# JVBSouza/descriptools

Hardware: AMD Instinct MI355X
Metric: Mcells/s full descriptor chain (higher is better)
Workload: dtype f32; 1 GPU; 16384x16384 synthetic tilted-integer-fBm DEM per GPU, full chain (d8, flowacc, river mask, flowhand/HAND with fused GFI + ln(hl/H), fused slope+TI+MTI, downslope), device-resident; global_dem=16384x16384, river_threshold_cells=524288

## Files before the change

### descriptools_amd/csrc/dt_fa3fh1_kernel.inc

```
#if FA3_WALK
#define FA3_NAME(n) n##w
#define FA3_NAME_TWI(n) n##w_twi
#else
#define FA3_NAME(n) n
#define FA3_NAME_TWI(n) n##_twi
#endif
#if FA3_TWI
__global__ __launch_bounds__(256, 6) void FA3_NAME_TWI(k_fa3fh1)(const uint8_t *__restrict__ fdr, const float *__restrict__ dem,
#else
template <int ND>
__global__ __launch_bounds__(256, 6) void FA3_NAME(k_fa3fh1)(const uint8_t *__restrict__ fdr, const float *__restrict__ dem,
#endif
                                                  const uint8_t *__restrict__ nod4, int ldm, DtWin w, int tiles_x,
                                                  const unsigned long long *__restrict__ rec,
                                                  const unsigned long long *__restrict__ state,
                                                  const unsigned long long *__restrict__ ext,
                                                  const uint16_t *__restrict__ loc16, int32_t *__restrict__ acc32,
                                                  int32_t river_thr, int8_t *__restrict__ river,
                                                  int *__restrict__ status, uint32_t nnodes,
                                                  unsigned long long *__restrict__ nodes,
                                                  unsigned long long *__restrict__ cache,
#if FA3_TWI
                                                  uint8_t *__restrict__ cache_wide, TwiOut tw) {
  constexpr int ND = 2;
#else
                                                  uint8_t *__restrict__ cache_wide) {
#endif
#undef FA3_NAME
#undef FA3_NAME_TWI
#define P3(c) ((uint32_t)(c) + (((uint32_t)(c) >> 6) << 2))
#define NT3 (TH * (TW + 4))
  __shared__ __attribute__((aligned(16))) unsigned char smem[NT3 * 6];
  __shared__ unsigned long long s_in;
#if !FA3_WALK
  __shared__ int s_ovf;
#endif
  uint32_t *s_delta = reinterpret_cast<uint32_t *>(smem);
  uint16_t *s_nxt = reinterpret_cast<uint16_t *>(smem + NT3 * 4);
  const int tile = dt_tile_of_block((int)blockIdx.x, (int)gridDim.x);
  const int ty = tile / tiles_x, tx = tile - ty * tiles_x;
  const int y0 = ty * TH, x0 = tx * TW;
  const uint4 v_fdr = dt_tile_fetch16(fdr, w, y0, x0);
  uint32_t c2[8] = {0u, 0u, 0u, 0u, 0u, 0u, 0u, 0u};
  if (rec) fa_nbr_codes(fdr, w, y0, x0, threadIdx.x, c2);
  unsigned long long e = 0ull;
  if (threadIdx.x < PS && ext) e = ext[(size_t)tile * PS + threadIdx.x];
  constexpr int VPT = NT / 4 / 256;
  uint2 l4[VPT];
  float4 z4[VPT];
#if FA3_TWI
  fa_v4f s4[VPT];
#endif
#pragma unroll
  for (int u = 0; u < VPT; u++) {
    int c = 4 * (threadIdx.x + 256 * u);
    int y = y0 + c / TW;
    l4[u] = *reinterpret_cast<const uint2 *>(loc16 + (size_t)tile * NT + c);
    z4[u] = make_float4(0.f, 0.f, 0.f, 0.f);
#if FA3_TWI
    s4[u] = (fa_v4f){0.f, 0.f, 0.f, 0.f};
    if (y < w.H)
      s4[u] = __builtin_nontemporal_load(reinterpret_cast<const fa_v4f *>(tw.slope + (long long)y * w.ld + x0 + c % TW));
#endif
    if (ND == 1 && y < w.H) z4[u] = *reinterpret_cast<const float4 *>(dem + (long long)y * w.ld + x0 + c % TW);
    if (ND == 2 && y < w.H) {
      const uint32_t m = (uint32_t)reinterpret_cast<const uint16_t *>(nod4)[(long long)(y >> 2) * ldm + ((x0 + c % TW) >> 2)] >>
                         (4 * (y & 3));
      z4[u] = make_float4((m & 1u) ? DT_NODATA : 0.f, (m & 2u) ? DT_NODATA : 0.f, (m & 4u) ? DT_NODATA : 0.f,
                          (m & 8u) ? DT_NODATA : 0.f);
    }
  }
  {
    const int ly = (int)threadIdx.x >> 2, lxb = ((int)threadIdx.x & 3) * 16;
    const uint32_t cv[4] = {v_fdr.x, v_fdr.y, v_fdr.z, v_fdr.w};
    const bool interior = dt_tile_interior(w, y0, x0);
    const int pbase = ly * (TW + 4) + lxb;
#pragma unroll
    for (int q = 0; q < 4; q++) {
      uint32_t nn[4];
#pragma unroll
      for (int k = 0; k < 4; k++) {
        const uint32_t code = (cv[q] >> (8 * k)) & 0xFFu;
        const int lx = lxb + 4 * q + k;
        const uint32_t n = interior ? dt_tile_next_interior(code, ly, lx) : dt_tile_next(code, ly, lx, y0, x0, w);
        nn[k] = n < NT ? P3(n) : n;
      }
      *reinterpret_cast<uint2 *>(&s_nxt[pbase + 4 * q]) = make_uint2(nn[0] | (nn[1] << 16), nn[2] | (nn[3] << 16));
      *reinterpret_cast<uint4 *>(&s_delta[pbase + 4 * q]) = make_uint4(0, 0, 0, 0);
    }
  }
  if (rec) e = fa_inflow(fa_gather(c2, y0, x0, threadIdx.x, tiles_x, rec, state), e);
#if FA3_WALK
  bool fed_now = false;
#pragma unroll
  for (int q = 0; q < 8; q++) fed_now = fed_now || c2[q] == fa_back(q);
  const unsigned long long fed_mask = __ballot(fed_now);
#endif
#if !FA3_WALK
  if (threadIdx.x == 0) s_ovf = 0;
#endif
  if (__syncthreads_or(!(e & FA_CYCLE) && FA_VALUE(e) >= (1ull << 22))) {
    if (threadIdx.x == 0) s_in = 0ull;
    __syncthreads();
    if (e != 0ull && !(e & FA_CYCLE)) atomicAdd(&s_in, FA_VALUE(e));
    __syncthreads();
    if (threadIdx.x == 0 && s_in >= (1ull << 31) - (unsigned long long)NT && status) atomicOr(status, DT_STATUS_ACC_OVERFLOW);
  }
  if (e != 0ull) {
    int ly, lx;
    dt_cell_of_slot(threadIdx.x, ly, lx);
    uint32_t c = P3(ly * TW + lx);
    if (e & FA_CYCLE) {
      for (int it = 0; it < NT && c < NT3; it++) {
        atomicOr(&s_delta[c], 0x80000000u);
        c = s_nxt[c];
      }
    } else {
      const uint32_t add = (uint32_t)e;
      for (int it = 0; it < NT && c < NT3; it++) {
        atomicAdd(&s_delta[c], add);
        c = s_nxt[c];
      }
    }
  }
  __syncthreads();
  auto finish = [&](uint32_t l16, uint32_t d, float z) -> int32_t {
    int32_t v = l16 == 0xFFFFu ? -100 : (int32_t)l16;
    if (v != -100) v += (int32_t)(d & 0x7FFFFFFFu);
    if (d & 0x80000000u) v = -100;
    if (ND != 0 && z <= DT_NODATA) v = -100;
    return v;
  };
  uint32_t riv4[VPT];
#pragma unroll
  for (int u = 0; u < VPT; u++) {
    int c = 4 * (threadIdx.x + 256 * u);
    int y = y0 + c / TW;
    riv4[u] = 0u;
    if (y >= w.H) continue;
    long long o = (long long)y * w.ld + x0 + c % TW;
    uint4 d = *reinterpret_cast<const uint4 *>(&s_delta[P3(c)]);
    int4 v = make_int4(finish(l4[u].x & 0xFFFFu, d.x, z4[u].x), finish(l4[u].x >> 16, d.y, z4[u].y),
                       finish(l4[u].y & 0xFFFFu, d.z, z4[u].z), finish(l4[u].y >> 16, d.w, z4[u].w));
    *reinterpret_cast<int4 *>(acc32 + o) = v;
    riv4[u] = (v.x > river_thr ? 1u : 0u) | (v.y > river_thr ? 0x100u : 0u) | (v.z > river_thr ? 0x10000u : 0u) |
              (v.w > river_thr ? 0x1000000u : 0u);
    *reinterpret_cast<uint32_t *>(river + o) = riv4[u];
#if FA3_TWI
    {
      const int32_t fv[4] = {v.x, v.y, v.z, v.w};
      const double nlnpx2 = tw.n_top * tw.lnpx2;
      fa_v4f tio, mtio;
      uint32_t rej = 0u;
#pragma unroll
      for (int k = 0; k < 4; k++) {
        const float q = dt_pct_to_tan(s4[u][k]);
        const bool tnod = fv[k] <= -100;
        float tv, mv;
        rej |= ((sd_twi_fast(fv[k], q, tw.n_top, tw.lnpx2, nlnpx2, tv, mv) && !tnod) ? 1u : 0u) << k;
        tio[k] = tnod ? DT_NODATA : tv;
        mtio[k] = tnod ? DT_NODATA : mv;
      }
      __builtin_nontemporal_store(tio, reinterpret_cast<fa_v4f *>(tw.ti + o));
      __builtin_nontemporal_store(mtio, reinterpret_cast<fa_v4f *>(tw.mti + o));
      if (rej) {
        const int x = x0 + c % TW;
        const int stile = (y >> 4) * tw.stiles_x + (x >> 8);
        const size_t lane = (size_t)stile * 256 + (size_t)(((y & 15) >> 2) * 64 + ((x & 255) >> 2));
        atomicOr(&tw.lane_mask[lane >> 1], rej << (16 * (int)(lane & 1) + 4 * (y & 3)));
        tw.tile_mark[stile] = (uint8_t)1;
      }
    }
#endif
  }
#if FA3_WALK
#pragma unroll
  for (int u = 0; u < VPT; u++) {
    if (!riv4[u]) continue;
    const uint32_t pc = P3(4 * (threadIdx.x + 256 * u));
    uint2 nx = *reinterpret_cast<const uint2 *>(&s_nxt[pc]);
    if (riv4[u] & 0x1u) nx.x = (nx.x & 0xFFFF0000u) | NX_RIVER;
    if (riv4[u] & 0x100u) nx.x = (nx.x & 0xFFFFu) | (NX_RIVER << 16);
    if (riv4[u] & 0x10000u) nx.y = (nx.y & 0xFFFF0000u) | NX_RIVER;
    if (riv4[u] & 0x1000000u) nx.y = (nx.y & 0xFFFFu) | (NX_RIVER << 16);
    *reinterpret_cast<uint2 *>(&s_nxt[pc]) = nx;
  }
#endif
  __syncthreads();
#if FA3_WALK
  fh_walk_body(s_nxt, fdr, ((fed_mask >> (threadIdx.x & 63u)) & 1ull) != 0ull, w, tile, tiles_x, y0, x0, nodes, cache_wide);
#undef P3
#undef NT3
}
#else
#undef P3
#undef NT3
  uint32_t *s_w = reinterpret_cast<uint32_t *>(smem);
  uint8_t *s_fdr = smem + NT * 4;
  uint8_t *s_kind = smem + NT * 5;
  uint32_t *s_lut = reinterpret_cast<uint32_t *>(smem + NT * 6);
  s_lut[threadIdx.x] = fh_lut_entry(threadIdx.x);
  dt_tile_put16(s_fdr, v_fdr);
  __syncthreads();
  fh_tile1n_body(s_fdr, s_w, s_kind, &s_ovf, s_lut, riv4, w, tile, tiles_x, y0, x0, nnodes, nodes, cache, cache_wide);
}
#endif
```

### descriptools_amd/csrc/dt_tiles.hip

```cpp
#include "dt_common.h"
#include "dt_kernels.h"
#include "dt_math.h"

#define TW 64
#define TH 64
#define NT (TW * TH)
#define PS (2 * TW + 2 * (TH - 2))
#define CPT (NT / 256)

#define NX_SINK 0xFFFFu
#define NX_EXIT 0xFFFEu
#define NX_REXIT 0xFFFDu
#define X_NONE 0xFFFFu

__device__ __forceinline__ int dt_slot_of(int ly, int lx) {
  if (ly == 0) return lx;
  if (ly == TH - 1) return TW + lx;
  if (lx == 0) return 2 * TW + (ly - 1);
  if (lx == TW - 1) return 2 * TW + (TH - 2) + (ly - 1);
  return -1;
}
__device__ __forceinline__ void dt_cell_of_slot(int s, int &ly, int &lx) {
  if (s < TW) { ly = 0; lx = s; }
  else if (s < 2 * TW) { ly = TH - 1; lx = s - TW; }
// ... 1122 lines not shown
      if (y >= w.H || x >= w.W || code == 0u) {
        s = fht_pack((uint32_t)c | (K_DEAD << 12), 0, FHT_DONE);
      } else if ((riv >> j) & 1u) {
        s = fht_pack((uint32_t)c | (K_RIVER << 12), 0, FHT_DONE);
      } else if (!dt_d8_valid(code)) {
        s = fht_pack((uint32_t)c | (K_DEAD << 12), 0, FHT_DONE);
      } else {
        int dy, dx;
        dt_d8_delta(code, dy, dx);
        int ty = y + dy, tx = x + dx;
        if (!dt_in_global(w, ty, tx) || fht_fdr_at(T, ly + dy, lx + dx) == 0u) {
          s = fht_pack((uint32_t)c | (K_DEAD << 12), 0, FHT_DONE);
        } else if (!dt_in_core(w, ty, tx)) {
          s = fht_pack((uint32_t)c | (K_REXIT << 12), 0, FHT_DONE);
        } else if (ly + dy < 0 || ly + dy >= TH || lx + dx < 0 || lx + dx >= TW) {
          s = fht_pack((uint32_t)c | (K_EXIT << 12), 0, FHT_DONE);
        } else {
          bool diag = dy != 0 && dx != 0;
          s = fht_pack((uint32_t)((ly + dy) * TW + lx + dx), diag ? 1u : 0u, diag ? 0u : 1u);
        }
      }
      T.s_st[c] = s;
    }
  }
  __syncthreads();
  ulonglong2 *s_st2 = reinterpret_cast<ulonglong2 *>(T.s_st);
  for (int round = 0; round < 13; round++) {
    int changed = 0;
#pragma unroll
    for (int j = 0; j < CPT / 2; j++) {
      int c2 = threadIdx.x + 256 * j;
      ulonglong2 s = s_st2[c2];
      bool dx = ((uint32_t)s.x & FHT_DONE) != 0u, dy = ((uint32_t)s.y & FHT_DONE) != 0u;
      if (dx && dy) continue;
      if (!dx) {
        unsigned long long t = T.s_st[(uint32_t)(s.x >> 32) & 0xFFFu];
        s.x = (t & 0xFFFFFFFF00000000ull) | (unsigned long long)((uint32_t)s.x + (uint32_t)t);
      }
      if (!dy) {
        unsigned long long t = T.s_st[(uint32_t)(s.y >> 32) & 0xFFFu];
        s.y = (t & 0xFFFFFFFF00000000ull) | (unsigned long long)((uint32_t)s.y + (uint32_t)t);
      }
      s_st2[c2] = s;
      changed |= (((uint32_t)s.x & (uint32_t)s.y & FHT_DONE) == 0u) ? 1 : 0;
    }
    if (!__syncthreads_or(changed)) break;
  }
#pragma unroll
  for (int j = 0; j < CPT; j++) {
    int c = threadIdx.x + 256 * j;
    if (!((uint32_t)T.s_st[c] & FHT_DONE)) T.s_st[c] = fht_pack((uint32_t)c | (K_DEAD << 12), 0, FHT_DONE);
  }
  __syncthreads();
}

__device__ __forceinline__ uint32_t fh_cache_pack(unsigned long long s) {
  uint32_t ptr = (uint32_t)(s >> 32);
  return (ptr & 0x7FFFu) | ((uint32_t)((s >> 16) & 0xFFu) << 15) | ((uint32_t)(s & 0xFFu) << 23);
}
__device__ __forceinline__ unsigned long long fh_cache_unpack(uint32_t v) {
  return fht_pack(v & 0x7FFFu, (v >> 15) & 0xFFu, ((v >> 23) & 0xFFu) | FHT_DONE);
}
__device__ __forceinline__ unsigned long long fh_cache_get(const unsigned long long *__restrict__ cache, bool wide,
                                                            int tile, int c) {
  if (wide) return cache[(size_t)tile * NT + c];
  return fh_cache_unpack(reinterpret_cast<const uint32_t *>(cache + (size_t)tile * NT)[c]);
}

template <bool NODES>
__device__ __forceinline__ void fh_tile1_tile(uint8_t *s_fdr, uint8_t *s_halo, unsigned long long *s_st, int tile,
                                              const uint8_t *__restrict__ fdr, const int8_t *__restrict__ river,
                                              const DtWin &w, int tiles_x, uint32_t nnodes,
                                              unsigned long long *__restrict__ nodes,
                                              unsigned long long *__restrict__ cache,
                                              uint8_t *__restrict__ cache_wide) {
  const int ty = tile / tiles_x, tx = tile - ty * tiles_x;
  const int y0 = ty * TH, x0 = tx * TW;
  FhTile T{s_fdr, s_halo, s_st};
  fht_solve_tile(T, fdr, river, w, y0, x0);
  if (NODES && threadIdx.x < PS) {
    int ly, lx;
    dt_cell_of_slot(threadIdx.x, ly, lx);
    unsigned long long s = s_st[ly * TW + lx];
    uint32_t ptr = (uint32_t)(s >> 32), nd = (uint32_t)((s >> 16) & 0xFFFFu);
    uint32_t ncf = (uint32_t)(s & 0xFFFFu), nc = ncf & 0x7FFFu;
    uint32_t kind = (ptr >> 12) & 7u, f = ptr & 0xFFFu;
    int fy = (int)f / TW, fx = (int)f % TW;
    unsigned long long o = fht_pack(FHT_DEAD, 0, FHT_DONE);
    if (!(ncf & FHT_DONE)) {
    } else if (kind == K_RIVER) {
      o = fht_pack((uint32_t)((y0 + fy) * w.W + x0 + fx), nd, nc | FHT_DONE);
    } else if (kind == K_EXIT || kind == K_REXIT) {
      int dy, dx;
      dt_d8_delta(s_fdr[f], dy, dx);
      bool diag = dy != 0 && dx != 0;
      uint32_t node = kind == K_EXIT ? dt_node_of(y0 + fy + dy, x0 + fx + dx, tiles_x)
                                     : nnodes + (uint32_t)dt_perim_index(w.H, w.W, y0 + fy, x0 + fx);
      o = fht_pack(node, nd + (diag ? 1u : 0u), nc + (diag ? 0u : 1u));
    }
    nodes[(size_t)tile * PS + threadIdx.x] = o;
  }
  unsigned long long wv[CPT];
  int wide = 0;
#pragma unroll
  for (int j = 0; j < CPT; j++) {
    wv[j] = s_st[threadIdx.x + 256 * j];
    wide |= (((uint32_t)wv[j] & 0x7FFFu) > 255u || ((uint32_t)(wv[j] >> 16) & 0xFFFFu) > 255u) ? 1 : 0;
  }
  wide = __syncthreads_or(wide);
  if (threadIdx.x == 0) cache_wide[tile] = (uint8_t)wide;
  if (wide) {
#pragma unroll
    for (int j = 0; j < CPT; j++) cache[(size_t)tile * NT + threadIdx.x + 256 * j] = wv[j];
  } else {
    uint32_t *c32 = reinterpret_cast<uint32_t *>(cache + (size_t)tile * NT);
#pragma unroll
    for (int j = 0; j < CPT; j++) c32[threadIdx.x + 256 * j] = fh_cache_pack(wv[j]);
  }
  __syncthreads();
}
__global__ __launch_bounds__(256) void k_fh_tile1(const uint8_t *__restrict__ fdr,
                                                 const int8_t *__restrict__ river, DtWin w, int tiles_x,
                                                 uint32_t nnodes, unsigned long long *__restrict__ nodes,
                                                 unsigned long long *__restrict__ cache,
                                                 uint8_t *__restrict__ cache_wide, int only_marked, int ntiles) {
  __shared__ __attribute__((aligned(16))) uint8_t s_fdr[NT];
  __shared__ uint8_t s_halo[2 * (TW + 2) + 2 * TH];
  __shared__ __attribute__((aligned(16))) unsigned long long s_st[NT];
  for (int tile = (int)blockIdx.x; tile < ntiles; tile += (int)gridDim.x) {
    if (only_marked && cache_wide[tile] != 2) continue;
    fh_tile1_tile<true>(s_fdr, s_halo, s_st, tile, fdr, river, w, tiles_x, nnodes, nodes, cache, cache_wide);
  }
}
__global__ __launch_bounds__(256) void k_fh_tile1_marked(const uint8_t *__restrict__ fdr,
                                                        const int8_t *__restrict__ river, DtWin w, int tiles_x,
                                                        uint32_t nnodes, unsigned long long *__restrict__ nodes,
                                                        unsigned long long *__restrict__ cache,
                                                        uint8_t *cache_wide, int ntiles) {
  __shared__ __attribute__((aligned(16))) uint8_t s_fdr[NT];
  __shared__ uint8_t s_halo[2 * (TW + 2) + 2 * TH];
  __shared__ __attribute__((aligned(16))) unsigned long long s_st[NT];
  __shared__ uint8_t s_flag[256];
  const int base = (int)blockIdx.x * 256, mine = base + (int)threadIdx.x;
  const uint8_t flag = mine < ntiles ? cache_wide[mine] : (uint8_t)0;
  s_flag[threadIdx.x] = flag;
  if (!__syncthreads_or(flag == 2)) return;
  for (int i = 0; i < 256; i++)
    if (s_flag[i] == 2)
      fh_tile1_tile<false>(s_fdr, s_halo, s_st, base + i, fdr, river, w, tiles_x, nnodes, nodes, cache, cache_wide);
}

#define FN_CNT 0x3FFFFu
#define FN_DONE 0x40000u
#define FN_LOW 0x7FFFFu
#define FN_OVF 0x20100u
#define FN_PTR_SH 19
__device__ __forceinline__ uint32_t fh_lut_entry(uint32_t code) {
  if (!dt_d8_valid(code)) return 0u;
  int dy, dx;
  dt_d8_delta(code, dy, dx);
  return ((uint32_t)(dy * TW + dx) << FN_PTR_SH) + ((dy != 0 && dx != 0) ? (1u << 9) : 1u);
}
__device__ __forceinline__ bool fh_tile1n_solve(uint8_t *s_fdr, uint32_t *s_w, uint8_t *s_kind, int *s_ovf_p,
                                                const uint32_t *s_lut, const uint32_t (&riv4)[NT / 4 / 256],
                                                const DtWin &w, int y0, int x0, uint2 (&own)[CPT / 2]) {
#define s_ovf (*s_ovf_p)
  const bool interior = dt_tile_interior(w, y0, x0);
  const uint32_t lx0 = (4u * threadIdx.x) & 63u;
#pragma unroll
  for (int u = 0; u < NT / 4 / 256; u++) {
    const int c0 = 4 * (threadIdx.x + 256 * u);
    const uint32_t codes = *reinterpret_cast<const uint32_t *>(&s_fdr[c0]);
    uint32_t wd[4], kinds = 0;
#pragma unroll
    for (int k = 0; k < 4; k++) {
      const int c = c0 + k;
      const uint32_t code = (codes >> (8 * k)) & 0xFFu, cw = (uint32_t)c << FN_PTR_SH;
      const bool is_river = ((riv4[u] >> (8 * k)) & 0xFFu) == 1u;
      uint32_t word = cw | FN_DONE, kind = K_DEAD;
      if (interior) {
        const uint32_t wn = cw + s_lut[code];
        if (code != 0u) {
          if (is_river) {
            kind = K_RIVER;
          } else if (wn & FN_CNT) {
            const bool out = (int32_t)wn < 0 || (((wn >> FN_PTR_SH) & 63u) - (lx0 + (uint32_t)k - 1u)) > 2u;
            if (out) kind = K_EXIT;
            else word = wn;
          }
        }
      } else {
        const int ly = c / TW, lx = c % TW;
        const int y = y0 + ly, x = x0 + lx;
        if (y < w.H && x < w.W && code != 0u) {
          if (is_river) {
            kind = K_RIVER;
          } else if (dt_d8_valid(code)) {
            int dy, dx;
            dt_d8_delta(code, dy, dx);
            uint32_t ny = (uint32_t)(ly + dy), nx = (uint32_t)(lx + dx);
            bool in_tile = ny < (uint32_t)TH && nx < (uint32_t)TW;
            if (dt_in_global(w, y + dy, x + dx)) {
              if (!dt_in_core(w, y + dy, x + dx)) kind = K_REXIT;
              else if (!in_tile) kind = K_EXIT;
              else word = ((ny * TW + nx) << FN_PTR_SH) | ((dy != 0 && dx != 0) ? (1u << 9) : 1u);
            }
          }
        }
      }
      wd[k] = word;
      kinds |= kind << (8 * k);
    }
    *reinterpret_cast<uint4 *>(&s_w[c0]) = make_uint4(wd[0], wd[1], wd[2], wd[3]);
    *reinterpret_cast<uint32_t *>(&s_kind[c0]) = kinds;
  }
  __syncthreads();
  uint2 *s_w2 = reinterpret_cast<uint2 *>(s_w);
#pragma unroll
  for (int j = 0; j < CPT / 2; j++) own[j] = s_w2[threadIdx.x + 256 * j];
  for (int round = 0; round < 13; round++) {
    int changed = 0;
    uint32_t ovf = 0;
#pragma unroll
    for (int j = 0; j < CPT / 2; j++) {
      int c2 = threadIdx.x + 256 * j;
      uint2 v = own[j];
      bool dx = (v.x & FN_DONE) != 0u, dy = (v.y & FN_DONE) != 0u;
      if (dx && dy) continue;
      if (!dx) {
        v.x = s_w[v.x >> FN_PTR_SH] + (v.x & FN_CNT);
        if (!(v.x & (FN_DONE | FN_OVF))) v.x = s_w[v.x >> FN_PTR_SH] + (v.x & FN_CNT);
        ovf |= v.x & FN_OVF;
      }
      if (!dy) {
        v.y = s_w[v.y >> FN_PTR_SH] + (v.y & FN_CNT);
        if (!(v.y & (FN_DONE | FN_OVF))) v.y = s_w[v.y >> FN_PTR_SH] + (v.y & FN_CNT);
        ovf |= v.y & FN_OVF;
      }
      own[j] = v;
      s_w2[c2] = v;
      changed |= ((v.x & v.y & FN_DONE) == 0u) ? 1 : 0;
    }
    if (ovf) s_ovf = 1;
    if (!__syncthreads_or(changed)) break;
    if (s_ovf) break;
  }
  return !s_ovf;
#undef s_ovf
}
__device__ __forceinline__ uint32_t fh_narrow_word(uint32_t v, uint32_t c, const uint8_t *s_kind) {
  uint32_t f = v >> FN_PTR_SH, kind = s_kind[f];
  if (!(v & FN_DONE)) { f = c; kind = K_DEAD; v = 0; }
  return f | (kind << 12) | (((v >> 9) & 0xFFu) << 15) | ((v & 0xFFu) << 23);
}
__device__ __forceinline__ void fh_tile1n_body(uint8_t *s_fdr, uint32_t *s_w, uint8_t *s_kind, int *s_ovf_p,
                                               const uint32_t *s_lut, const uint32_t (&riv4)[NT / 4 / 256],
                                               const DtWin &w, int tile, int tiles_x, int y0, int x0, uint32_t nnodes,
                                               unsigned long long *__restrict__ nodes,
                                               unsigned long long *__restrict__ cache,
                                               uint8_t *__restrict__ cache_wide) {
  uint2 own[CPT / 2];
  if (!fh_tile1n_solve(s_fdr, s_w, s_kind, s_ovf_p, s_lut, riv4, w, y0, x0, own)) {
    if (threadIdx.x == 0) cache_wide[tile] = 2;
    return;
  }
  uint2 *s_w2 = reinterpret_cast<uint2 *>(s_w);
  auto narrow = [&](uint32_t v, uint32_t c) -> uint32_t { return fh_narrow_word(v, c, s_kind); };
#pragma unroll
  for (int j = 0; j < CPT / 2; j++) {
    const int c2 = threadIdx.x + 256 * j;
    s_w2[c2] = make_uint2(narrow(own[j].x, 2u * (uint32_t)c2), narrow(own[j].y, 2u * (uint32_t)c2 + 1u));
  }
  if (threadIdx.x == 0) cache_wide[tile] = 0;
  __syncthreads();
  uint32_t *c32 = reinterpret_cast<uint32_t *>(cache + (size_t)tile * NT);
#pragma unroll
  for (int u = 0; u < NT / 4 / 256; u++) {
    int c = 4 * (threadIdx.x + 256 * u);
    *reinterpret_cast<uint4 *>(c32 + c) = *reinterpret_cast<const uint4 *>(&s_w[c]);
  }
  if (threadIdx.x < PS) {
    int ly, lx;
    dt_cell_of_slot(threadIdx.x, ly, lx);
    unsigned long long sw = fh_cache_unpack(s_w[ly * TW + lx]);
    uint32_t ptr = (uint32_t)(sw >> 32), nd = (uint32_t)((sw >> 16) & 0xFFFFu), nc = (uint32_t)sw & 0x7FFFu;
    uint32_t kind = (ptr >> 12) & 7u, f = ptr & 0xFFFu;
    int fy = (int)f / TW, fx = (int)f % TW;
    unsigned long long o = fht_pack(FHT_DEAD, 0, FHT_DONE);
    if (kind == K_RIVER) {
      o = fht_pack((uint32_t)((y0 + fy) * w.W + x0 + fx), nd, nc | FHT_DONE);
    } else if (kind == K_EXIT || kind == K_REXIT) {
      int dy, dx;
      dt_d8_delta(s_fdr[f], dy, dx);
      bool diag = dy != 0 && dx != 0;
      uint32_t node = kind == K_EXIT ? dt_node_of(y0 + fy + dy, x0 + fx + dx, tiles_x)
                                     : nnodes + (uint32_t)dt_perim_index(w.H, w.W, y0 + fy, x0 + fx);
      o = fht_pack(node, nd + (diag ? 1u : 0u), nc + (diag ? 0u : 1u));
    }
    nodes[(size_t)tile * PS + threadIdx.x] = o;
  }
}

#define NX_RIVER 0xFFFCu
#define FH_SOLVE_LATER 3
__device__ __forceinline__ void fh_walk_body(const uint16_t *s_nxt, const uint8_t *__restrict__ fdr, bool fed, const DtWin &w,
                                             int tile, int tiles_x, int y0, int x0,
                                             unsigned long long *__restrict__ nodes,
                                             uint8_t *__restrict__ cache_wide) {
  constexpr uint32_t PW = TW + 4, NTP = TH * PW;
  if (threadIdx.x == 0) cache_wide[tile] = (uint8_t)FH_SOLVE_LATER;
  if (threadIdx.x >= PS) return;
  unsigned long long o = fht_pack(FHT_DEAD, 0, FHT_DONE);
  if (fed) {
    int ly, lx;
    dt_cell_of_slot(threadIdx.x, ly, lx);
    uint32_t c = (uint32_t)ly * PW + (uint32_t)lx, nc = 0, nd = 0;
    uint32_t n = 0;
    for (int it = 0; it < NT; it++) {
      n = s_nxt[c];
      if (n >= NTP) break;
      const uint32_t d = n > c ? n - c : c - n;
      if (d == 1u || d == PW) nc++;
      else nd++;
      c = n;
    }
    if (n == NX_RIVER || n == NX_EXIT) {
      const int fy = (int)(c / PW), fx = (int)(c % PW);
      const uint32_t code = fdr[(long long)(y0 + fy) * w.ld + x0 + fx];
      if (n == NX_EXIT) {
        int dy, dx;
        dt_d8_delta(code, dy, dx);
        const bool diag = dy != 0 && dx != 0;
        o = fht_pack(dt_node_of(y0 + fy + dy, x0 + fx + dx, tiles_x), nd + (diag ? 1u : 0u), nc + (diag ? 0u : 1u));
      } else if (code != 0u) {
        o = fht_pack((uint32_t)((y0 + fy) * w.W + x0 + fx), nd, nc | FHT_DONE);
      }
    }
  }
  nodes[(size_t)tile * PS + threadIdx.x] = o;
}

__global__ __launch_bounds__(256, 6) void k_fh_tile1n(const uint8_t *__restrict__ fdr,
                                                     const int8_t *__restrict__ river, DtWin w, int tiles_x,
                                                     uint32_t nnodes, unsigned long long *__restrict__ nodes,
                                                     unsigned long long *__restrict__ cache,
                                                     uint8_t *__restrict__ cache_wide) {
  __shared__ __attribute__((aligned(16))) uint8_t s_fdr[NT];
  __shared__ __attribute__((aligned(16))) uint32_t s_w[NT];
  __shared__ __attribute__((aligned(16))) uint8_t s_kind[NT];
  __shared__ uint32_t s_lut[256];
  __shared__ int s_ovf;
  const int tile = dt_tile_of_block((int)blockIdx.x, (int)gridDim.x);
  const int ty = tile / tiles_x, tx = tile - ty * tiles_x;
  const int y0 = ty * TH, x0 = tx * TW;
  const uint4 v_fdr = dt_tile_fetch16(fdr, w, y0, x0);
  const uint4 v_riv = dt_tile_fetch16(reinterpret_cast<const uint8_t *>(river), w, y0, x0);
  dt_tile_put16(s_fdr, v_fdr);
  dt_tile_put16(s_kind, v_riv);
  s_lut[threadIdx.x] = fh_lut_entry(threadIdx.x);
  if (threadIdx.x == 0) s_ovf = 0;
  __syncthreads();
  uint32_t riv4[NT / 4 / 256];
#pragma unroll
  for (int u = 0; u < NT / 4 / 256; u++) riv4[u] = *reinterpret_cast<const uint32_t *>(&s_kind[4 * (threadIdx.x + 256 * u)]);
  fh_tile1n_body(s_fdr, s_w, s_kind, &s_ovf, s_lut, riv4, w, tile, tiles_x, y0, x0, nnodes, nodes, cache, cache_wide);
}


struct TwiOut {
  const float *slope;
  float *ti, *mti;
  double n_top, lnpx2;
  uint8_t *tile_mark;
  uint32_t *lane_mask;
  int stiles_x;
};
typedef float fa_v4f __attribute__((ext_vector_type(4)));
#define FA3_WALK 0
#define FA3_TWI 0
#include "dt_fa3fh1_kernel.inc"
#undef FA3_TWI
#define FA3_TWI 1
#include "dt_fa3fh1_kernel.inc"
#undef FA3_TWI
#undef FA3_WALK
#define FA3_WALK 1
#define FA3_TWI 0
#include "dt_fa3fh1_kernel.inc"
#undef FA3_TWI
#define FA3_TWI 1
#include "dt_fa3fh1_kernel.inc"
#undef FA3_TWI
#undef FA3_WALK

__global__ __launch_bounds__(256) void k_fh_ghost_init(unsigned long long *__restrict__ nodes, uint32_t nnodes,
                                                      int64_t P) {
  int64_t i = (int64_t)blockIdx.x * 256 + threadIdx.x;
  if (i < P) nodes[nnodes + i] = fht_pack(nnodes + (uint32_t)i, 0, 0);
}

__global__ __launch_bounds__(256) void k_fh_node_jump(unsigned long long *__restrict__ state, int64_t n,
                                                      int *__restrict__ flags, int round, int hops) {
  if (flags && round > 0 && flags[round - 1] == 0) {
    if (blockIdx.x == 0 && threadIdx.x == 0) flags[round] = 0;
    return;
  }
  bool pending = false;
  for (int64_t i = (int64_t)blockIdx.x * 256 + threadIdx.x; i < n; i += (int64_t)gridDim.x * 256) {
    unsigned long long s = __hip_atomic_load(&state[i], __ATOMIC_RELAXED, __HIP_MEMORY_SCOPE_AGENT);
    bool open = false, changed = false;
    for (int h = 0; h < hops; h++) {
      const uint32_t ncf = (uint32_t)(s & 0xFFFFu);
      const uint32_t ptr = (uint32_t)(s >> 32), nd = (uint32_t)((s >> 16) & 0xFFFFu);
      if ((ncf & FHT_DONE) || ptr == (uint32_t)i) break;
      const unsigned long long t = __hip_atomic_load(&state[ptr], __ATOMIC_RELAXED, __HIP_MEMORY_SCOPE_AGENT);
      const uint32_t tptr = (uint32_t)(t >> 32), tnd = (uint32_t)((t >> 16) & 0xFFFFu);
      const uint32_t tncf = (uint32_t)(t & 0xFFFFu);
      const uint32_t nnc = ncf + (tncf & 0x7FFFu), nnd = nd + tnd;
      if (((tncf & FHT_DONE) && tptr == FHT_DEAD) || nnc + nnd > FHT_CAP) s = fht_pack(FHT_DEAD, 0, FHT_DONE);
      else s = fht_pack(tptr, nnd, nnc | (tncf & FHT_DONE));
      changed = true;
      open = !(s & (unsigned long long)FHT_DONE) && tptr != ptr;
      if (!open) break;
    }
    if (changed) __hip_atomic_store(&state[i], s, __ATOMIC_RELAXED, __HIP_MEMORY_SCOPE_AGENT);
    pending = pending || open;
  }
  if (flags && __any(pending) && (threadIdx.x & 63) == 0) flags[round] = 1;
}

template <typename AccT>
__global__ __launch_bounds__(256) void k_fh_rank_summary(DtWin w, int tiles_x, uint32_t nnodes,
                                                        const unsigned long long *__restrict__ nodes,
                                                        const float *__restrict__ dem,
                                                        const AccT *__restrict__ acc32, int64_t P,
                                                        uint8_t *__restrict__ kind, int32_t *__restrict__ ref,
                                                        int32_t *__restrict__ nc, int32_t *__restrict__ nd,
                                                        float *__restrict__ zr, long long *__restrict__ ar) {
  int64_t i = (int64_t)blockIdx.x * 256 + threadIdx.x;
  if (i >= P) return;
  int y, x;
  dt_perim_cell(w.H, w.W, i, y, x);
  const bool has_node = dt_slot_of(y % TH, x % TW) >= 0;
  unsigned long long s = has_node ? nodes[dt_node_of(y, x, tiles_x)] : fht_pack(FHT_DEAD, 0, FHT_DONE);
  uint32_t ptr = (uint32_t)(s >> 32), ncf = (uint32_t)(s & 0xFFFFu);
  uint8_t k = (uint8_t)K_DEAD;
  int32_t r = -1;
  float z = DT_NODATA;
  long long a = 0;
  if (ncf & FHT_DONE) {
    if (ptr != FHT_DEAD) {
      k = (uint8_t)K_RIVER;
      r = (int32_t)ptr;
      long long o = (long long)(ptr / (uint32_t)w.W) * w.ld + (ptr % (uint32_t)w.W);
      if (dem) z = dem[o];
      if (acc32) a = (long long)acc32[o];
    }
  } else if (ptr >= nnodes) {
    k = (uint8_t)K_REXIT;
    r = (int32_t)(ptr - nnodes);
  }
  kind[i] = k;
  ref[i] = r;
  nc[i] = (int32_t)(ncf & 0x7FFFu);
  nd[i] = (int32_t)((s >> 16) & 0xFFFFu);
  zr[i] = z;
  ar[i] = a;
}

__global__ __launch_bounds__(256) void k_fh_ghost_set(unsigned long long *__restrict__ nodes, uint32_t nnodes,
                                                     int64_t P, const uint8_t *__restrict__ res_ok,
                                                     const int32_t *__restrict__ res_nc,
                                                     const int32_t *__restrict__ res_nd) {
  int64_t i = (int64_t)blockIdx.x * 256 + threadIdx.x;
  if (i >= P) return;
  unsigned long long o = fht_pack(FHT_DEAD, 0, FHT_DONE);
  if (res_ok[i]) o = fht_pack(FHT_REMOTE | (uint32_t)i, (uint32_t)res_nd[i], (uint32_t)res_nc[i] | FHT_DONE);
  nodes[nnodes + i] = o;
}

struct FhGfi {
  float *gfi, *lnhlh;
  double expo, c0;
  const DtLogEntry *tab;
};
struct FhRemote {
  const long long *gidx;
  const float *zr;
  const long long *ar;
};
template <typename AccT>
struct FhPay;
template <>
struct FhPay<int32_t> {
  unsigned long long v[PS];
  __device__ __forceinline__ void set(int i, float z, int32_t a) {
    v[i] = ((unsigned long long)(uint32_t)a << 32) | (unsigned long long)__float_as_uint(z);
  }
  __device__ __forceinline__ void get(int i, float &z, int32_t &a) const {
    const unsigned long long p = v[i];
    z = __uint_as_float((uint32_t)p);
    a = (int32_t)(uint32_t)(p >> 32);
  }
};
template <>
struct FhPay<long long> {
  long long av[PS];
  float zv[PS];
  __device__ __forceinline__ void set(int i, float z, long long a) {
    av[i] = a;
    zv[i] = z;
  }
  __device__ __forceinline__ void get(int i, float &z, long long &a) const {
    z = zv[i];
    a = av[i];
  }
};

typedef float fh_v4f __attribute__((ext_vector_type(4)));
typedef int fh_v4i __attribute__((ext_vector_type(4)));
__device__ __forceinline__ void fh_store4(float *p, float a, float b, float c, float d) {
  fh_v4f v = {a, b, c, d};
  __builtin_nontemporal_store(v, reinterpret_cast<fh_v4f *>(p));
}
__device__ __forceinline__ void fh_store4(int32_t *p, int32_t a, int32_t b, int32_t c, int32_t d) {
  fh_v4i v = {a, b, c, d};
  __builtin_nontemporal_store(v, reinterpret_cast<fh_v4i *>(p));
}
typedef long long fh_v2l __attribute__((ext_vector_type(2)));
__device__ __forceinline__ void fh_store4(long long *p, long long a, long long b, long long c, long long d) {
  fh_v2l v0 = {a, b}, v1 = {c, d};
  __builtin_nontemporal_store(v0, reinterpret_cast<fh_v2l *>(p));
  __builtin_nontemporal_store(v1, reinterpret_cast<fh_v2l *>(p + 2));
}

struct FhSolveLds {
  uint8_t *fdr;
  uint32_t *w;
  uint8_t *kind;
  uint32_t *lut;
  int *ovf;
  double *term;
};
template <bool RANKED, int VH, typename AccT, bool SOLVE>
__device__ __forceinline__ bool fh_tile3_tile(unsigned long long *s_x, FhPay<AccT> &s_pay, DtLogEntry *s_tab,
                                              const FhSolveLds &L, const int8_t *__restrict__ river, int tile,
                                              const uint8_t *__restrict__ fdr, const float *__restrict__ dem,
                                              const AccT *__restrict__ acc32, const DtWin &w, int tiles_x,
                                              uint32_t nnodes, const unsigned long long *__restrict__ nodes,
                                              const unsigned long long *__restrict__ cache, bool wide,
                                              const FhRemote &rem, double px, float *__restrict__ fdist,
                                              int32_t *__restrict__ idx32, long long *__restrict__ idx64,
                                              float *__restrict__ hand, AccT *__restrict__ a_river,
                                              const FhGfi &G) {
  const int ty = tile / tiles_x, tx = tile - ty * tiles_x;
  const int y0 = ty * TH, x0 = tx * TW;
  const bool vec = x0 + TW <= w.W && (w.ld & 3) == 0 && (!dem || ((uintptr_t)dem & 15) == 0) &&
                   (!fdist || ((uintptr_t)fdist & 15) == 0) && (!idx32 || ((uintptr_t)idx32 & 15) == 0) &&
                   (!idx64 || ((uintptr_t)idx64 & 15) == 0) && (!hand || ((uintptr_t)hand & 15) == 0) &&
                   (!a_river || ((uintptr_t)a_river & 15) == 0) &&
                   (!G.gfi || ((((uintptr_t)G.gfi | (uintptr_t)G.lnhlh | (uintptr_t)acc32) & 15) == 0));
  [[maybe_unused]] auto load_z4 = [&](int u) -> float4 {
    const int c = 4 * (threadIdx.x + 256 * u), y = y0 + c / TW;
    float4 z = make_float4(DT_NODATA, DT_NODATA, DT_NODATA, DT_NODATA);
    if (dem && y < w.H) z = *reinterpret_cast<const float4 *>(dem + (long long)y * w.ld + x0 + c % TW);
    return z;
  };
  [[maybe_unused]] auto load_f4 = [&](int u) -> int4 {
    const int c = 4 * (threadIdx.x + 256 * u), y = y0 + c / TW;
    int4 f = make_int4(0, 0, 0, 0);
    if (G.gfi && y < w.H) f = *reinterpret_cast<const int4 *>(acc32 + (long long)y * w.ld + x0 + c % TW);
    return f;
  };
  float4 z4_first = make_float4(DT_NODATA, DT_NODATA, DT_NODATA, DT_NODATA);
  int4 f4_first = make_int4(0, 0, 0, 0);
  int slot_ly = 0, slot_lx = 0;
  if (threadIdx.x < PS) dt_cell_of_slot(threadIdx.x, slot_ly, slot_lx);
  uint32_t slot_code = 0;
  bool has_river = true;
  if (SOLVE) {
    const uint4 v_fdr = dt_tile_fetch16(fdr, w, y0, x0);
    const uint4 v_riv = dt_tile_fetch16(reinterpret_cast<const uint8_t *>(river), w, y0, x0);
    if (vec) {
      z4_first = load_z4(0);
      f4_first = load_f4(0);
    }
    dt_tile_put16(L.fdr, v_fdr);
    dt_tile_put16(L.kind, v_riv);
    L.lut[threadIdx.x] = fh_lut_entry(threadIdx.x);
    if (threadIdx.x == 0) *L.ovf = 0;
    has_river = __syncthreads_or((v_riv.x | v_riv.y | v_riv.z | v_riv.w) != 0u) != 0;
    if (threadIdx.x < PS) slot_code = L.fdr[slot_ly * TW + slot_lx];
    uint32_t riv4[NT / 4 / 256];
#pragma unroll
    for (int u = 0; u < NT / 4 / 256; u++) riv4[u] = *reinterpret_cast<const uint32_t *>(&L.kind[4 * (threadIdx.x + 256 * u)]);
    uint2 own[CPT / 2];
    if (!fh_tile1n_solve(L.fdr, L.w, L.kind, L.ovf, L.lut, riv4, w, y0, x0, own)) return false;
  }
  auto solved = [&](uint32_t v, int c) -> uint32_t { return fh_narrow_word(v, (uint32_t)c, L.kind); };
  if (threadIdx.x < PS) {
    const int ly = slot_ly, lx = slot_lx;
    int f = ly * TW + lx;
    bool ex, rex;
    if (SOLVE) {
      const uint32_t v = L.w[f];
      const bool self = (v & FN_DONE) != 0u && (v >> FN_PTR_SH) == (uint32_t)f;
      const uint32_t kind = L.kind[f];
      ex = self && kind == K_EXIT;
      rex = self && kind == K_REXIT;
    } else {
      const uint32_t sp = (uint32_t)(fh_cache_get(cache, wide, tile, f) >> 32);
      ex = sp == ((uint32_t)f | (K_EXIT << 12));
      rex = sp == ((uint32_t)f | (K_REXIT << 12));
    }
    unsigned long long o = fht_pack(FHT_DEAD, 0, FHT_DONE);
    float zr = DT_NODATA;
    AccT ar = -100;
    if (ex || rex) {
      int dy, dx;
      dt_d8_delta(SOLVE ? slot_code : (uint32_t)fdr[(long long)(y0 + ly) * w.ld + x0 + lx], dy, dx);
      size_t node = ex ? (size_t)dt_node_of(y0 + ly + dy, x0 + lx + dx, tiles_x)
                       : (size_t)nnodes + (size_t)dt_perim_index(w.H, w.W, y0 + ly, x0 + lx);
      unsigned long long ns = nodes[node];
      uint32_t nptr = (uint32_t)(ns >> 32), nnd = (uint32_t)((ns >> 16) & 0xFFFFu);
      uint32_t nncf = (uint32_t)(ns & 0xFFFFu);
      if (RANKED && !(nncf & FHT_DONE) && nptr >= nnodes && (size_t)nptr != node) {
        unsigned long long gs = nodes[nptr];
        uint32_t gncf = (uint32_t)(gs & 0xFFFFu);
        nnd += (uint32_t)((gs >> 16) & 0xFFFFu);
        const uint32_t cnt = (nncf & 0x7FFFu) + (gncf & 0x7FFFu);
        nptr = (uint32_t)(gs >> 32);
        if ((gncf & FHT_DONE) && nptr != FHT_DEAD && cnt + nnd <= FHT_CAP) nncf = cnt | FHT_DONE;
        else nptr = FHT_DEAD;
      }
      bool diag = dy != 0 && dx != 0;
      if ((nncf & FHT_DONE) && nptr != FHT_DEAD) {
        o = fht_pack(nptr, nnd + (diag ? 1u : 0u), ((nncf & 0x7FFFu) + (diag ? 0u : 1u)) | FHT_DONE);
        if (RANKED && (nptr & FHT_REMOTE)) {
          zr = rem.zr[nptr & ~FHT_REMOTE];
// ... 800 lines not shown
```

Baseline: 37790 Mcells/s.

## Fuse HAND perimeter walk into flow-accumulation walk and encode diag/exit in successor

Packs a diagonal bit and the exit direction code into each 16-bit successor word so a walk can count diagonal and cardinal steps and resolve exits without re-reading fdr from global memory. When a tile has no river cells, the perimeter node words for fed slots are emitted during the existing flow-accumulation walk, and the second HAND walk is skipped for those slots. This removes a redundant per-slot walk and a global fdr load, in exchange for extra bit masking in the hot loop, a shared river flag, and tighter encoding constraints on tile size.

```diff
diff --git a/descriptools_amd/csrc/dt_fa3fh1_kernel.inc b/descriptools_amd/csrc/dt_fa3fh1_kernel.inc
--- a/descriptools_amd/csrc/dt_fa3fh1_kernel.inc
+++ b/descriptools_amd/csrc/dt_fa3fh1_kernel.inc
@@ -37,6 +37,9 @@
 #endif
   uint32_t *s_delta = reinterpret_cast<uint32_t *>(smem);
   uint16_t *s_nxt = reinterpret_cast<uint16_t *>(smem + NT3 * 4);
+#if FA3_WALK
+  constexpr int W_RIVER_FLAG = TW;
+#endif
   const int tile = dt_tile_of_block((int)blockIdx.x, (int)gridDim.x);
   const int ty = tile / tiles_x, tx = tile - ty * tiles_x;
   const int y0 = ty * TH, x0 = tx * TW;
@@ -83,11 +86,28 @@
         const uint32_t code = (cv[q] >> (8 * k)) & 0xFFu;
         const int lx = lxb + 4 * q + k;
         const uint32_t n = interior ? dt_tile_next_interior(code, ly, lx) : dt_tile_next(code, ly, lx, y0, x0, w);
+#if FA3_WALK
+        nn[k] = n < NT ? P3(n) : n == NX_EXIT ? (NX_EXIT_CODE | code) : n;
+#else
         nn[k] = n < NT ? P3(n) : n;
-      }
+#endif
+      }
+#if FA3_WALK
+      uint32_t dg = cv[q] & 0xAAAAAAAAu;
+      dg |= dg >> 2;
+      dg |= dg >> 4;
+      static_assert(NX_DIAG == (2u << 12), "the fold below puts bit 1 of a byte on NX_DIAG");
+      nn[0] |= (dg & 0x2u) << 12;
+      nn[1] |= (dg & 0x200u) << 4;
+      nn[2] |= (dg & 0x20000u) >> 4;
+      nn[3] |= (dg & 0x2000000u) >> 12;
+#endif
       *reinterpret_cast<uint2 *>(&s_nxt[pbase + 4 * q]) = make_uint2(nn[0] | (nn[1] << 16), nn[2] | (nn[3] << 16));
       *reinterpret_cast<uint4 *>(&s_delta[pbase + 4 * q]) = make_uint4(0, 0, 0, 0);
     }
+#if FA3_WALK
+    if (threadIdx.x == 0) s_delta[W_RIVER_FLAG] = 0u;
+#endif
   }
   if (rec) e = fa_inflow(fa_gather(c2, y0, x0, threadIdx.x, tiles_x, rec, state), e);
 #if FA3_WALK
@@ -106,6 +126,9 @@
     __syncthreads();
     if (threadIdx.x == 0 && s_in >= (1ull << 31) - (unsigned long long)NT && status) atomicOr(status, DT_STATUS_ACC_OVERFLOW);
   }
+#if FA3_WALK
+  bool w_have = false;
+#endif
   if (e != 0ull) {
     int ly, lx;
     dt_cell_of_slot(threadIdx.x, ly, lx);
@@ -113,16 +136,39 @@
     if (e & FA_CYCLE) {
       for (int it = 0; it < NT && c < NT3; it++) {
         atomicOr(&s_delta[c], 0x80000000u);
+#if FA3_WALK
+        c = s_nxt[c] & NX_CELL;
+#else
         c = s_nxt[c];
+#endif
       }
     } else {
       const uint32_t add = (uint32_t)e;
+#if FA3_WALK
+      uint32_t came = 0u, acc = ~0u, n = 0u;
+      for (int it = 0; it < NT; it++) {
+        atomicAdd(&s_delta[c], add);
+        n = s_nxt[c];
+        acc += fh_count(came);
+        if (n > NX_CELL_MAX) break;
+        came = n;
+        c = n & NX_CELL;
+      }
+      if (n > NX_CELL_MAX) {
+        w_have = true;
+        nodes[(size_t)tile * PS + threadIdx.x] = fh_walk_word(n, c, acc, tiles_x, y0, x0);
+      }
+#else
       for (int it = 0; it < NT && c < NT3; it++) {
         atomicAdd(&s_delta[c], add);
         c = s_nxt[c];
       }
-    }
-  }
+#endif
+    }
+  }
+#if FA3_WALK
+  const unsigned long long word_mask = __ballot(w_have) & fed_mask;
+#endif
   __syncthreads();
   auto finish = [&](uint32_t l16, uint32_t d, float z) -> int32_t {
     int32_t v = l16 == 0xFFFFu ? -100 : (int32_t)l16;
@@ -185,14 +231,21 @@
     if (riv4[u] & 0x1000000u) nx.y = (nx.y & 0xFFFFu) | (NX_RIVER << 16);
     *reinterpret_cast<uint2 *>(&s_nxt[pc]) = nx;
   }
-#endif
-  __syncthreads();
-#if FA3_WALK
-  fh_walk_body(s_nxt, fdr, ((fed_mask >> (threadIdx.x & 63u)) & 1ull) != 0ull, w, tile, tiles_x, y0, x0, nodes, cache_wide);
+  {
+    bool has_river = false;
+#pragma unroll
+    for (int u = 0; u < VPT; u++) has_river = has_river || riv4[u] != 0u;
+    if (has_river) s_delta[W_RIVER_FLAG] = 1u;
+  }
+  __syncthreads();
+  const unsigned long long keep_mask = s_delta[W_RIVER_FLAG] != 0u ? 0ull : word_mask;
+  fh_walk_body(s_nxt, fdr, ((fed_mask >> (threadIdx.x & 63u)) & 1ull) != 0ull,
+               ((keep_mask >> (threadIdx.x & 63u)) & 1ull) != 0ull, w, tile, tiles_x, y0, x0, nodes, cache_wide);
 #undef P3
 #undef NT3
 }
 #else
+  __syncthreads();
 #undef P3
 #undef NT3
   uint32_t *s_w = reinterpret_cast<uint32_t *>(smem);
diff --git a/descriptools_amd/csrc/dt_tiles.hip b/descriptools_amd/csrc/dt_tiles.hip
--- a/descriptools_amd/csrc/dt_tiles.hip
+++ b/descriptools_amd/csrc/dt_tiles.hip
@@ -1448,39 +1448,50 @@
 }
 
 #define NX_RIVER 0xFFFCu
+#define NX_EXIT_CODE 0xFF00u
+#define NX_DIAG 0x2000u
+#define NX_CELL 0x1FFFu
+#define NX_CELL_MAX 0x3FFFu
 #define FH_SOLVE_LATER 3
-__device__ __forceinline__ void fh_walk_body(const uint16_t *s_nxt, const uint8_t *__restrict__ fdr, bool fed, const DtWin &w,
-                                             int tile, int tiles_x, int y0, int x0,
+__device__ __forceinline__ uint32_t fh_count(uint32_t word) { return (word & NX_DIAG) + 1u; }
+__device__ __forceinline__ unsigned long long fh_walk_word(uint32_t n, uint32_t c, uint32_t acc, int tiles_x, int y0,
+                                                           int x0) {
+  constexpr uint32_t PW = TW + 4;
+  static_assert(TH * PW - 1 <= NX_CELL && (NX_DIAG | NX_CELL) == NX_CELL_MAX && NX_CELL_MAX < NX_EXIT_CODE &&
+                (NX_EXIT_CODE | 0x80u) < NX_RIVER, "successor word");
+  if (n <= NX_CELL_MAX || n >= NX_RIVER) return fht_pack(FHT_DEAD, 0, FHT_DONE);
+  const uint32_t nd = acc >> 13, nc = (acc & NX_CELL) - nd;
+  int dy, dx;
+  dt_d8_delta(n & 0xFFu, dy, dx);
+  const bool diag = dy != 0 && dx != 0;
+  return fht_pack(dt_node_of(y0 + (int)(c / PW) + dy, x0 + (int)(c % PW) + dx, tiles_x), nd + (diag ? 1u : 0u),
+                  nc + (diag ? 0u : 1u));
+}
+__device__ __forceinline__ void fh_walk_body(const uint16_t *s_nxt, const uint8_t *__restrict__ fdr, bool fed, bool keep,
+                                             const DtWin &w, int tile, int tiles_x, int y0, int x0,
                                              unsigned long long *__restrict__ nodes,
                                              uint8_t *__restrict__ cache_wide) {
-  constexpr uint32_t PW = TW + 4, NTP = TH * PW;
+  constexpr uint32_t PW = TW + 4;
   if (threadIdx.x == 0) cache_wide[tile] = (uint8_t)FH_SOLVE_LATER;
-  if (threadIdx.x >= PS) return;
+  if (threadIdx.x >= PS || keep) return;
   unsigned long long o = fht_pack(FHT_DEAD, 0, FHT_DONE);
   if (fed) {
     int ly, lx;
     dt_cell_of_slot(threadIdx.x, ly, lx);
-    uint32_t c = (uint32_t)ly * PW + (uint32_t)lx, nc = 0, nd = 0;
+    uint32_t c = (uint32_t)ly * PW + (uint32_t)lx, acc = 0;
     uint32_t n = 0;
     for (int it = 0; it < NT; it++) {
       n = s_nxt[c];
-      if (n >= NTP) break;
-      const uint32_t d = n > c ? n - c : c - n;
-      if (d == 1u || d == PW) nc++;
-      else nd++;
-      c = n;
-    }
-    if (n == NX_RIVER || n == NX_EXIT) {
+      if (n > NX_CELL_MAX) break;
+      acc += fh_count(n);
+      c = n & NX_CELL;
+    }
+    if (n == NX_RIVER) {
       const int fy = (int)(c / PW), fx = (int)(c % PW);
-      const uint32_t code = fdr[(long long)(y0 + fy) * w.ld + x0 + fx];
-      if (n == NX_EXIT) {
-        int dy, dx;
-        dt_d8_delta(code, dy, dx);
-        const bool diag = dy != 0 && dx != 0;
-        o = fht_pack(dt_node_of(y0 + fy + dy, x0 + fx + dx, tiles_x), nd + (diag ? 1u : 0u), nc + (diag ? 0u : 1u));
-      } else if (code != 0u) {
-        o = fht_pack((uint32_t)((y0 + fy) * w.W + x0 + fx), nd, nc | FHT_DONE);
-      }
+      if (fdr[(long long)(y0 + fy) * w.ld + x0 + fx] != 0u)
+        o = fht_pack((uint32_t)((y0 + fy) * w.W + x0 + fx), acc >> 13, ((acc & NX_CELL) - (acc >> 13)) | FHT_DONE);
+    } else {
+      o = fh_walk_word(n, c, acc, tiles_x, y0, x0);
     }
   }
   nodes[(size_t)tile * PS + threadIdx.x] = o;
```

Result: faster. 38320 Mcells/s (median of 6 runs) (+1.4%).
